# Fannovel16/stylish-tts

Hardware: AMD Instinct MI355X
Metric: utterances_per_sec (higher is better)
Workload: dtype f32; 1 GPU; cfg2: LJSpeech-shaped batch=8 x 3.0 s per GPU (T=240 mel frames, 72000 samples @24 kHz) fp32, Decoder + PriorEncoder/reverse flow + freegan iSTFT vocoder (stts_frame_path); no diffusion step exists in the reference; batch_per_gpu=8, global_batch=8, frames_per_utt=960, parallelism=single GPU, ranks=1, backend=none, distinct_devices=1

## Files before the change

### stylish_tts_amd/csrc/model.hip.h

```cpp
#pragma once
#include <math.h>

#include <array>
#include <map>
#include <memory>
#include <mutex>
#include <string>
#include <vector>

#include "../../include/stylish_hip.h"
#include "common.h"
#include "elementwise.hip.h"
#include "gemm.hip.h"
#include "gemm16.hip.h"
#include "signal.hip.h"
#include "signal_geom.hip.h"
#include "phoneme.hip.h"
#include "wn_layer.hip.h"
#include "wn_layer_small.hip.h"
#include "wn_fused.hip.h"
#include "wn_fused16.hip.h"
#include "wn_block16.hip.h"
#include "wn_fused_x3.hip.h"
#include "wn_block_x3.hip.h"
// ... 742 lines not shown
}
#define STTS_DRY_RETURN(arena)                                                   \
  do {                                                                            \
    if (stts::dry_run().on) {                                                     \
      stts::dry_run().peak = std::max(stts::dry_run().peak, (arena).offset0 + (arena).used); \
      return 0;                                                                   \
    }                                                                             \
  } while (0)

struct Arena {
  char* base;
  size_t cap, used = 0;
  size_t offset0 = 0;
  bool ok = true;
  Arena(void* p, size_t n, size_t off0 = 0) : base((char*)p), cap(n), offset0(off0) {}
  template <typename T>
  T* get(size_t count) {
    const size_t bytes = (count * sizeof(T) + 255) / 256 * 256;
    if (used + bytes > cap) {
      ok = false;
      return nullptr;
    }
    T* p = (T*)(base + used);
    used += bytes;
    return p;
  }
};

struct Seg {
  int n_utt;
  const int* host;
  const int* dev;
  bool cap = false;
  const int* rows_dev() const { return cap ? dev + n_utt : nullptr; }
  int rows() const { return host[n_utt]; }
  int max_len() const {
    int m = 0;
    for (int i = 0; i < n_utt; ++i) m = std::max(m, host[i + 1] - host[i]);
    return m;
  }
};

inline GemmArgs gemm_args(const Seg& s) {
  GemmArgs a;
  memset(&a, 0, sizeof(a));
  a.seg_off = s.dev;
  a.seg_host = s.host;
  a.n_utt = s.n_utt;
  a.rows_total = s.rows();
  a.capacity = s.cap;
  if (!s.cap && s.host && s.n_utt > 0) {
    const int len = s.host[1] - s.host[0];
    bool same = len > 0;
    for (int u = 1; u < s.n_utt && same; ++u) same = s.host[u + 1] - s.host[u] == len;
    if (same) { a.uniform_len = len; a.uniform_lo0 = s.host[0]; }
  }
  a.alpha = 1.0f;
  a.xaff_slope = 0.2f;
  a.zeros = zero_page();
  return a;
}
inline void set_seg(GemmArgs& a, int i, const float* X, int ldx, int xcol0, const PackedConv& w, int pad = -1, int dil = 1) {
  GemmSeg& g = a.seg[i];
  g.X = X;
  g.W = w.W;
  g.W16 = w.W16;
  g.w16_plane = w.w16_plane;
  if (i == 0) a.prec = w.prec;
  g.w_utt_stride = 0;
  g.ldx = ldx;
  g.xcol0 = xcol0;
  g.kc = w.kc;
  g.ntaps = w.ntaps;
  g.dil = dil;
  g.pad = pad >= 0 ? pad : (w.ntaps - 1) / 2;
  g.kreal = w.cin_real;
  if (i == 0) a.wrows = w.rows_real;
  if (a.nseg < i + 1) a.nseg = i + 1;
}

struct WinoScratch {
  float* p = nullptr;
  bool setup = false;
  explicit operator bool() const { return p != nullptr; }
};
inline size_t wino_scratch_floats(const Seg& s, const WinoConv& wc) {
  const long pr = wino_plane_rows(s.rows(), s.n_utt);
  return (size_t)wc.mats.n * pr * (wc.planes.kc * 3 / 2 + round_up(wc.planes.N, 32)) + round_up(s.n_utt + 1 + 16, 32) + 32;
}
template <int N>
inline int run_winograd_n(hipStream_t st, const Seg& s, const float* X, int ldx, const WinoConv& wc, float* Y, int ldy, int act, const float* R, int ldr,
                          float alpha, WinoScratch& scratch, const float* aff = nullptr, int ld_aff = 0, float* stat = nullptr, int ld_stat = 0) {
  const int n = wc.mats.n, kc = wc.planes.kc, ldm = round_up(wc.planes.N, 32), ml = s.max_len();
  long pr = 0;
  for (int u = 0; u < s.n_utt; ++u) pr += ceil_div(s.host[u + 1] - s.host[u], kWinoM);
  const long pr_cap = wino_plane_rows(s.rows(), s.n_utt);
  int* segp = reinterpret_cast<int*>(scratch.p);
  int* goff = segp + 16;
  float* Xp = scratch.p + round_up(s.n_utt + 1 + 16, 32);
  static const bool presplit_env = getenv("STTS_X3_PRESPLIT") && atoi(getenv("STTS_X3_PRESPLIT")) != 0;
  const bool presplit = presplit_env && x3_enabled() && wc.planes.w16_plane > 0 && wc.planes.prec == PREC_F32 && kc % 8 == 0;
  const long xplane = (long)n * pr_cap * kc;
  float* Mp = Xp + (size_t)n * pr_cap * kc * 3 / 2;
  WinoIn ti;
  WinoOut to;
  memcpy(ti.Bt, wc.mats.Bt, sizeof(ti.Bt));
  memcpy(to.At, wc.mats.At, sizeof(to.At));
  const int groups = ceil_div(ml, kWinoM);
  GemmProfiler& prof = gemm_profiler();
  const bool timed = prof.on;
  if (timed) {
    (void)hipEventRecord(prof.next(), st);
    prof.on = false;
  }
  if (!scratch.setup) {
    hipLaunchKernelGGL(wino_setup_kernel, dim3(1), dim3(64), 0, st, s.dev, s.n_utt, kWinoMaxN, goff, segp);
    scratch.setup = true;
  }
  if (presplit)
    hipLaunchKernelGGL((winograd_input_kernel<N, true>), dim3(ceil_div(groups, 4), ceil_div(kc / 4, 64), s.n_utt), dim3(64, 4), 0, st, X, ldx,
                       wc.planes.cin_real, s.dev, wc.pad, ti, Xp, kc, goff, aff, ld_aff, xplane);
  else
  hipLaunchKernelGGL((winograd_input_kernel<N>), dim3(ceil_div(groups, 4), ceil_div(kc / 4, 64), s.n_utt), dim3(64, 4), 0, st, X, ldx,
                     wc.planes.cin_real, s.dev, wc.pad, ti, Xp, kc, goff, aff, ld_aff, 0L);
  std::vector<int> seg_h(n + 1);
  for (int j = 0; j <= n; ++j) seg_h[j] = (int)(j * pr);
  Seg sp{n, seg_h.data(), segp};
  sp.cap = s.cap;
  GemmArgs a = gemm_args(sp);
  set_seg(a, 0, Xp, kc, 0, wc.planes, 0);
  a.seg[0].w_utt_stride = (long)wc.planes.npad * kc;
  if (presplit) {
    a.x16 = 1;
    a.seg[0].x_plane = xplane;
  }
  a.N = wc.planes.N; a.bias = nullptr; a.Y = Mp; a.ldy = ldm;
  {
    const int rc = launch_conv_gemm(st, a, EPI_STORE, wc.planes.npad, n, (int)pr);
    if (rc) {
      prof.on = timed;
      return rc;
    }
  }
  if (stat)
    hipLaunchKernelGGL((winograd_output_kernel<N, true>), dim3(ceil_div(groups, 4), ceil_div(ceil_div(wc.planes.N, 4), 64), s.n_utt), dim3(64, 4), 0, st, Mp, ldm, goff,
                       s.dev, to, wc.planes.bias, act, R, ldr, alpha, Y, ldy, wc.planes.N, stat, ld_stat, ceil_div(groups, 4));
  else
    hipLaunchKernelGGL((winograd_output_kernel<N, false>), dim3(ceil_div(groups, 4), ceil_div(ceil_div(wc.planes.N, 4), 64), s.n_utt), dim3(64, 4), 0, st, Mp, ldm, goff,
                       s.dev, to, wc.planes.bias, act, R, ldr, alpha, Y, ldy, wc.planes.N, nullptr, 0, 0);
  if (timed) {
    prof.on = true;
    (void)hipEventRecord(prof.next(), st);
    prof.add((x3_enabled() && wc.planes.w16_plane > 0) ? "winograd_conv_x3" : "winograd_conv", 0, 2.0 * (double)s.rows() * wc.planes.rows_real * wc.planes.cin_real * wc.mats.r,
             2.0 * (double)n * (double)pr * wc.planes.rows_real * wc.planes.cin_real, 0.0);
  }
  STTS_HIP(hipGetLastError());
  return 0;
}
inline int wino_stat_chunks(const Seg& s) { return ceil_div(ceil_div(s.max_len(), kWinoM), 4); }
inline int run_winograd(hipStream_t st, const Seg& s, const float* X, int ldx, const WinoConv& wc, float* Y, int ldy, int act, const float* R, int ldr,
                        float alpha, WinoScratch& scratch, const float* aff = nullptr, int ld_aff = 0, float* stat = nullptr, int ld_stat = 0) {
  STTS_CHECK(wc.ready && (wc.mats.n == 8 || wc.mats.n == 12), "winograd conv not packed");
  STTS_CHECK(ldx % 4 == 0 && ldy % 4 == 0 && (!R || ldr % 4 == 0), "winograd conv: leading dimensions must be multiples of 4");
  STTS_CHECK(!stat || (ld_stat % 4 == 0 && ld_stat >= round_up(wc.planes.N, 4)), "winograd conv: statistics rows of %d floats do not cover %d channels", ld_stat, wc.planes.N);
  return wc.mats.n == 8 ? run_winograd_n<8>(st, s, X, ldx, wc, Y, ldy, act, R, ldr, alpha, scratch, aff, ld_aff, stat, ld_stat)
                        : run_winograd_n<12>(st, s, X, ldx, wc, Y, ldy, act, R, ldr, alpha, scratch, aff, ld_aff, stat, ld_stat);
}

inline int run_style(hipStream_t st, const StyleTable& t, const float* style, int n_utt, float* out) {
  if (n_utt >= 16 && t.K % 4 == 0 && t.K <= 128) {
    STTS_LAUNCH_PROF("style_fc_batch_kernel", (size_t)t.J * (t.K + n_utt) * 4, style_fc_batch_kernel, dim3(ceil_div(t.J, 4)), dim3(256), st, t.W, t.b, style, out,
                     t.J, t.K, n_utt, t.K, t.ld());
    STTS_HIP(hipGetLastError());
    return 0;
  }
  STTS_LAUNCH_PROF("style_fc_kernel", (size_t)t.J * (t.K + n_utt) * 4, style_fc_kernel, dim3(ceil_div(t.J, 4)), dim3(256), st, t.W, t.b, style, out, t.J, t.K, n_utt, t.K, t.ld());
  STTS_HIP(hipGetLastError());
  return 0;
}

inline dim3 rows_grid(const Seg& s, int per_row_work) {
  const long total = (long)s.max_len() * per_row_work;
  return dim3((unsigned)std::min<long>(std::max<long>(1, ceil_div((int)std::min<long>(total, 1 << 30), 256)), 512), s.n_utt);
}

inline long rows16_threshold() {
  static const long v = getenv("STTS_ROWS16") ? atol(getenv("STTS_ROWS16")) : 3840;
  return v;
}

inline size_t adain_part_floats(const Seg& s, int C, int chunk_rows = kStatChunk) { return (size_t)s.n_utt * ceil_div(s.max_len(), chunk_rows) * 2 * round_up(C, 32); }
inline int run_adain(hipStream_t st, const Seg& s, const float* X, int ldx, int C, float* Y, int ldy, const float* style_out, int ld_style,
                     int gcol0, int act, const float* alpha, float* part, int out16 = 0, bool have_stats = false) {
  const int nchunk = ceil_div(s.max_len(), kStatChunk), ldp = round_up(C, 32);
  if (!have_stats)
    STTS_LAUNCH_PROF("adain_partial_kernel", (size_t)s.rows() * C * 4, adain_partial_kernel, dim3(ceil_div(C, 32), nchunk, s.n_utt), dim3(256), st, X, ldx, C, s.dev, part, ldp, nchunk, kStatChunk);
  const int rb = (long)ceil_div(ldy, 64) * ceil_div(s.rows(), 64) >= 4096 ? 256 : 64;
  STTS_LAUNCH_PROF("adain_apply_kernel", (size_t)s.rows() * (C * 4 + ldy * (out16 ? 2 : 4)), adain_apply_kernel, dim3(ceil_div(ldy, 64), ceil_div(s.max_len(), rb), s.n_utt), dim3(256), st, X, ldx, Y, ldy, C, s.dev,
                     part, ldp, nchunk, style_out, ld_style, gcol0, 1e-5f, act, alpha, out16, rb);
  STTS_HIP(hipGetLastError());
  return 0;
}

struct PendingReduce {
  SplitSrc src{};
  float* Y = nullptr;
  int ldy = 0;
};
inline void pending_from(PendingReduce* p, const SplitInfo& info, const GemmArgs& a) {
  p->src = SplitSrc{};
  if (info.ksplit > 1) {
    p->src = SplitSrc{info.partial, info.ksplit, info.slice_rows, info.ld_part, a.N, a.bias, a.act, a.R, a.ldr, a.rcol0, a.alpha};
    p->Y = a.Y + a.ycol0;
    p->ldy = a.ldy;
  }
}
inline int pending_finish(hipStream_t st, PendingReduce* p) {
  if (!p || !p->src.partial) return 0;
  const SplitSrc& r = p->src;
  const long work = (long)r.slice_rows * ((r.N + 3) / 4);
  STTS_LAUNCH_PROF("splitk_reduce_kernel", (size_t)work * 4 * 4 * (r.ksplit + 1), splitk_reduce_kernel, dim3((unsigned)std::min<long>(2048, (work + 255) / 256)), dim3(256), st, r.partial,
                   r.ksplit, r.slice_rows, 0, r.ld_part, r.N, r.bias, r.act, r.R, r.ldr, r.rcol0, r.alpha, p->Y, p->ldy, 0);
  p->src = SplitSrc{};
  STTS_HIP(hipGetLastError());
  return 0;
}
inline long fold_rows() {
  static const long v = getenv("STTS_FOLD_ROWS") ? atol(getenv("STTS_FOLD_ROWS")) : 2500;
  return v;
}
struct SideWork {
  hipStream_t stream = nullptr;
  hipEvent_t fork = nullptr, join = nullptr;
  float* out = nullptr;
};
struct AdainStats {
  float* in = nullptr;
  bool in_ready = false;
  float* mid = nullptr;
  float* out = nullptr;
  int out_ld = 0;
  bool out_ready = false;
  int chunk_rows = kStatChunk;
};
inline int run_adain_block(hipStream_t st, const Seg& s, const AdainBlockW& B, const float* style_out, int ld_style, const float* x, int ldx,
                           float* y, int ldy, float* act1, float* hbuf, float* act2, float* ss, int force_tile = 0, WinoScratch* wino = nullptr,
                           unsigned short* xs16 = nullptr, bool xs16_ready = false, unsigned short* y16 = nullptr, int ldy16 = 0,
                           AdainStats* stats = nullptr, PendingReduce* pend_in = nullptr, PendingReduce* pend_out = nullptr, const SideWork* side = nullptr) {
  const int ml = s.max_len();
  const bool fold = s.rows() <= (B.conv1.prec == PREC_F32 ? fold_rows() : 4096);
  STTS_CHECK(ldx >= B.kcin, "adain block: input leading dimension %d < padded channels %d", ldx, B.kcin);
  static const bool affine_lanes = getenv("STTS_AFFINE_SERIAL") == nullptr;
  auto affine = [&](const float* X, int ld, int C, int ld_aff, int gcol0, float* aff, PendingReduce* pend = nullptr) {
    const int nchunk = ceil_div(ml, kStatChunk), ldp = round_up(C, 32);
    if (pend && pend->src.partial) {
      STTS_LAUNCH_PROF("adain_partial_reduce_kernel", (size_t)s.rows() * C * 4 * (1 + pend->src.ksplit), adain_partial_reduce_kernel, dim3(ceil_div(C, 32), nchunk, s.n_utt), dim3(256), st,
                       const_cast<float*>(X), ld, C, s.dev, ss, ldp, nchunk, pend->src);
      pend->src = SplitSrc{};
    } else
    STTS_LAUNCH_PROF("adain_partial_kernel", (size_t)s.rows() * C * 4, adain_partial_kernel, dim3(ceil_div(C, 32), nchunk, s.n_utt), dim3(256), st, X, ld, C, s.dev, ss, ldp, nchunk, kStatChunk);
    if (affine_lanes)
      STTS_LAUNCH_PROF("adain_affine_lanes_kernel", (size_t)s.n_utt * nchunk * 2 * ldp * 4, adain_affine_lanes_kernel, dim3(ceil_div(ld_aff, 16), s.n_utt), dim3(256), st, ss, ldp, nchunk, s.dev, style_out, ld_style,
                       gcol0, C, 1e-5f, aff, ld_aff, kStatChunk);
    else
    STTS_LAUNCH_PROF("adain_affine_kernel", (size_t)s.n_utt * nchunk * 2 * ldp * 4, adain_affine_kernel, dim3(ceil_div(ld_aff, 64), s.n_utt), dim3(64), st, ss, ldp, nchunk, s.dev, style_out, ld_style, gcol0, C,
                       1e-5f, aff, ld_aff, kStatChunk);
  };
  GemmArgs a = gemm_args(s);
  PendingReduce pend_mid;
  if (pend_in && pend_in->src.partial) STTS_CHECK(pend_in->Y == x && pend_in->ldy == ldx, "adain block: the pending reduce does not belong to this input");
  if (!fold) STTS_TRY(pending_finish(st, pend_in));
  if (fold) {
    affine(x, ldx, B.cin, B.kcin, B.n1.col0, act1, pend_in);
    set_seg(a, 0, x, ldx, 0, B.conv1);
    a.xaff = act1;
    a.ld_xaff = B.kcin;
  }
  const bool wino1 = !fold && wino && *wino && B.w1.ready && force_tile == 0;
  static const bool wino2_sc = getenv("STTS_NO_WINO_CONV2SC") == nullptr;
  const bool wino2 = !fold && wino && *wino && B.w2.ready && (!B.sc.W || wino2_sc) && force_tile == 0;
  const bool wstats = stats && stats->chunk_rows == kWinoStatChunk && wino1 && wino2;
  auto affine_from = [&](const float* part, int C, int ld_aff, int gcol0, float* aff) {
    const int wch = wino_stat_chunks(s), ldp = round_up(C, 32);
    STTS_LAUNCH_PROF("adain_affine_lanes_kernel", (size_t)s.n_utt * wch * 2 * ldp * 4, adain_affine_lanes_kernel, dim3(ceil_div(ld_aff, 16), s.n_utt), dim3(256), st, part, ldp, wch, s.dev, style_out, ld_style,
                     gcol0, C, 1e-5f, aff, ld_aff, kWinoStatChunk);
  };
  const int h16 = (s.rows() >= rows16_threshold() && B.conv1.prec != PREC_F32 && force_tile == 0 && (!B.sc.W || xs16) && ldx % 8 == 0) ? B.conv1.prec : 0;
  const int nchunk = ceil_div(ml, kStatChunk);
  const bool fuse_stats = stats && h16 && !fold && !wino1 && !wino2;
  if (!fold && !wino1) {
    const bool ready = fuse_stats && stats->in_ready;
    STTS_TRY(run_adain(st, s, x, ldx, B.cin, act1, B.kcin, style_out, ld_style, B.n1.col0, ACT_LRELU, nullptr, ready ? stats->in : ss, h16, ready));
    set_seg(a, 0, act1, B.kcin, 0, B.conv1);
    a.x16 = h16 != 0;
  }
  if (stats) stats->out_ready = false;
  a.N = B.cout;
  a.bias = B.conv1.bias;
  a.Y = hbuf;
  a.ldy = B.cout;
  auto shortcut = [&](hipStream_t sst, float* out) -> int {
    GemmArgs g = gemm_args(s);
    set_seg(g, 0, x, ldx, 0, B.sc);
    g.N = B.cout; g.bias = nullptr; g.Y = out; g.ldy = B.cout;
    return launch_conv_gemm(sst, g, EPI_STORE, B.sc.npad, s.n_utt, ml, 0);
  };
  const bool sc_side = side && side->stream && side->out && wino1 && wino2 && B.sc.W && !gemm_profiler().on;
  if (sc_side) {
    STTS_HIP(hipEventRecord(side->fork, st));
    STTS_HIP(hipStreamWaitEvent(side->stream, side->fork, 0));
    const int rc = shortcut(side->stream, side->out);
    STTS_HIP(hipEventRecord(side->join, side->stream));
    if (rc) { (void)hipStreamWaitEvent(st, side->join, 0); return rc; }
  }
  if (wino1) {
    if (wstats && stats->in_ready) affine_from(stats->in, B.cin, B.kcin, B.n1.col0, act1);
    else affine(x, ldx, B.cin, B.kcin, B.n1.col0, act1);
    STTS_TRY(run_winograd(st, s, x, ldx, B.w1, hbuf, B.cout, ACT_NONE, nullptr, 0, 1.0f, *wino, act1, B.kcin, wstats ? stats->mid : nullptr, round_up(B.cout, 32)));
  } else {
    if (fuse_stats && gemm16_will_run(a, EPI_STORE, B.conv1.npad, s.n_utt)) {
      a.stat_part = stats->mid; a.ld_stat = round_up(B.cout, 32); a.stat_nchunk = nchunk;
    }
    SplitInfo info1{};
    if (fold) a.defer = &info1;
    STTS_TRY(launch_conv_gemm(st, a, EPI_STORE, B.conv1.npad, s.n_utt, ml, force_tile));
    if (fold) pending_from(&pend_mid, info1, a);
  }
  const bool mid_ready = a.stat_part != nullptr;
  GemmArgs b = gemm_args(s);
  if (fold) {
    affine(hbuf, B.cout, B.cout, B.cout, B.n2.col0, act2, &pend_mid);
    set_seg(b, 0, hbuf, B.cout, 0, B.conv2);
    b.xaff = act2;
    b.ld_xaff = B.cout;
  } else if (wino2) {
    if (wstats) affine_from(stats->mid, B.cout, B.cout, B.n2.col0, act2);
    else affine(hbuf, B.cout, B.cout, B.cout, B.n2.col0, act2);
  } else {
    STTS_TRY(run_adain(st, s, hbuf, B.cout, B.cout, act2, B.cout, style_out, ld_style, B.n2.col0, ACT_LRELU, nullptr, mid_ready ? stats->mid : ss, h16, mid_ready));
    set_seg(b, 0, act2, B.cout, 0, B.conv2);
    b.x16 = h16 != 0;
  }
  if (B.sc.W) {
    if (h16) {
      if (!xs16_ready) launch_cast_rows(st, h16, x, ldx, B.cin, xs16, ldx, s.rows());
      set_seg(b, 1, reinterpret_cast<const float*>(xs16), ldx, 0, B.sc);
    } else {
      set_seg(b, 1, x, ldx, 0, B.sc);
    }
  } else {
    b.R = x;
    b.ldr = ldx;
  }
  b.N = B.cout;
  b.bias = B.conv2.bias;
  b.Y = y;
  b.ldy = ldy;
  b.alpha = 0.70710678118654752440f;
  const bool y16_epi = y16 && h16 && !wino2;
  if (y16_epi) {
    b.Y16 = y16;
    b.ldy16 = ldy16;
  }
  if (wino2) {
    const float* res = x;
    int ld_res = ldx;
    if (B.sc.W && sc_side) {
      STTS_HIP(hipStreamWaitEvent(st, side->join, 0));
      res = side->out;
      ld_res = B.cout;
    } else if (B.sc.W) {
      STTS_TRY(shortcut(st, act1));
      res = act1;
      ld_res = B.cout;
    }
    const bool leave = wstats && stats->out;
    STTS_TRY(run_winograd(st, s, hbuf, B.cout, B.w2, y, ldy, ACT_NONE, res, ld_res, b.alpha, *wino, act2, B.cout, leave ? stats->out : nullptr, leave ? stats->out_ld : 0));
    if (leave) stats->out_ready = true;
  } else {
    if (fuse_stats && stats->out && gemm16_will_run(b, EPI_STORE, B.conv2.npad, s.n_utt)) {
      b.stat_part = stats->out; b.ld_stat = stats->out_ld; b.stat_nchunk = nchunk;
      stats->out_ready = true;
    }
    SplitInfo info2{};
    if (fold && pend_out && !y16) b.defer = &info2;
    STTS_TRY(launch_conv_gemm(st, b, EPI_STORE, B.conv2.npad, s.n_utt, ml, force_tile));
    if (fold && pend_out && !y16) pending_from(pend_out, info2, b);
  }
  if (y16 && !y16_epi) launch_cast_rows(st, B.conv1.prec, y, ldy, B.cout, y16, ldy16, s.rows(), B.cout);
  STTS_HIP(hipGetLastError());
  return 0;
}

inline int decoder_forward(stts_ctx* c, hipStream_t st, const Seg& s, const float* asr, int ld_asr, const float* pitch, const float* energy,
                           const float* style, float* x_out, int ld_x, Arena& ws, const SideWork* side_lane = nullptr) {
  const stts_model_dims& d = c->d;
  const long R = s.rows();
  const int ccat = d.dec_hidden + d.dec_residual + 2, ldcat = c->dec[1].kcin;
  const int cenc = d.inter_dim + 2, ldenc = c->dec[0].kcin;
  STTS_CHECK(ldcat >= ccat && ldenc >= cenc, "decoder_forward: packed widths %d / %d do not cover %d / %d channels", ldcat, ldenc, ccat, cenc);
  const int ldwide = std::max(ldenc, ldcat);
  float* enc_in = ws.get<float>(R * ldenc);
  float* xa = ws.get<float>(R * ldcat);
  float* xb = ws.get<float>(R * ldcat);
  float* act1 = ws.get<float>(R * ldwide);
  float* hbuf = ws.get<float>(R * d.dec_hidden);
  float* act2 = ws.get<float>(R * d.dec_hidden);
  float* ss = ws.get<float>(adain_part_floats(s, ldwide));
  float* ss_in = ws.get<float>(adain_part_floats(s, ldwide, kWinoStatChunk));
  float* ss_mid = ws.get<float>(adain_part_floats(s, ldwide, kWinoStatChunk));
  float* sty = ws.get<float>((size_t)s.n_utt * c->dec_style.ld());
  WinoScratch wino;
  if (R > fold_rows() && c->dec[1].w1.ready) wino.p = ws.get<float>(wino_scratch_floats(s, c->dec[1].w1));
  float* sc_out = wino.p && c->dec[1].sc.W ? ws.get<float>(R * d.dec_hidden) : nullptr;
  const bool x16 = R >= rows16_threshold() && c->prec != PREC_F32 && d.dec_hidden % 8 == 0;
  unsigned short* xs16a = x16 ? ws.get<unsigned short>(R * ldwide) : nullptr;
  unsigned short* xs16b = x16 ? ws.get<unsigned short>(R * ldwide) : nullptr;
  STTS_CHECK(ws.ok, "decoder_forward: workspace too small");
  STTS_DRY_RETURN(ws);
  STTS_TRY(run_style(st, c->dec_style, style, s.n_utt, sty));
  FrontArgs fa;
  fa.asr = asr; fa.ld_asr = ld_asr; fa.pitch = pitch; fa.energy = energy;
  for (int i = 0; i < 3; ++i) { fa.wf[i] = c->front_wf[i]; fa.wn[i] = c->front_wn[i]; }
  fa.bf = c->front_bf; fa.bn = c->front_bn;
  fa.enc_in = enc_in; fa.ld_enc = ldenc; fa.xa = xa; fa.xb = xb; fa.ld_x = ldcat;
  fa.c_asr = d.inter_dim; fa.c_hidden = d.dec_hidden; fa.c_res = d.dec_residual;
  STTS_LAUNCH_PROF("decoder_front_kernel", (size_t)R * (d.inter_dim + 2 + ldenc + 2 * 4) * 4, decoder_front_kernel, rows_grid(s, ldenc / 4), dim3(256), st, fa, s.dev);
  for (float* dst : {xa, xb}) {
    GemmArgs a = gemm_args(s);
    set_seg(a, 0, asr, ld_asr, 0, c->asr_res);
    a.N = d.dec_residual; a.bias = c->asr_res.bias; a.Y = dst; a.ldy = ldcat; a.ycol0 = d.dec_hidden;
    STTS_TRY(launch_conv_gemm(st, a, EPI_STORE, c->asr_res.npad, s.n_utt, s.max_len()));
  }
  const int lds = c->dec_style.ld();
  const int ctail = d.dec_hidden & ~7, ntail = ldcat - ctail;
  auto cast_tail = [&](const float* src, unsigned short* dst) {
    launch_cast_rows(st, c->prec, src + ctail, ldcat, ccat - ctail, dst + ctail, ldcat, R, ntail);
  };
  static const bool no_stat_fuse = getenv("STTS_NO_STAT_FUSE") != nullptr;
  static const bool no_wino_stats = getenv("STTS_NO_WINO_STATS") != nullptr;
  const bool wstat_mode = c->prec == PREC_F32 && wino && !no_wino_stats;
  const bool use_stats = (x16 && !no_stat_fuse) || wstat_mode;
  AdainStats stats;
  if (wstat_mode) stats.chunk_rows = kWinoStatChunk;
  stats.mid = ss_mid;
  stats.out = ss_in;
  stats.out_ld = round_up(ccat, 32);
  PendingReduce pend;
  STTS_TRY(run_adain_block(st, s, c->dec[0], sty, lds, enc_in, ldenc, xa, ldcat, act1, hbuf, act2, ss, 0, &wino, xs16b, false, xs16a, ldcat, use_stats ? &stats : nullptr,
                           nullptr, &pend));
  if (x16) {
    cast_tail(xa, xs16a);
    cast_tail(xb, xs16b);
  }
  bool const_ready = false;
  auto const_columns = [&]() -> int {
    if (!stats.out_ready || const_ready) return 0;
    const int nchunk = ceil_div(s.max_len(), stats.chunk_rows), cc0 = d.dec_hidden, ncst = ccat - cc0;
    STTS_CHECK(cc0 % 32 == 0, "decoder_forward: hidden_dim must be a multiple of 32");
    STTS_LAUNCH_PROF("adain_partial_kernel", (size_t)R * ncst * 4, adain_partial_kernel, dim3(ceil_div(ncst, 32), nchunk, s.n_utt), dim3(256), st, xa + cc0, ldcat, ncst, s.dev,
                     ss_in + cc0, stats.out_ld, nchunk, stats.chunk_rows);
    const_ready = true;
    return 0;
  };
  STTS_TRY(const_columns());
  float* cur = xa;
  float* nxt = xb;
  unsigned short* cur16 = xs16a;
  unsigned short* nxt16 = xs16b;
  static const long sc_side_min_rows = getenv("STTS_SC_SIDE_MIN_ROWS") ? atol(getenv("STTS_SC_SIDE_MIN_ROWS")) : 12000;
  SideWork side;
  if (side_lane && sc_out && R >= sc_side_min_rows) {
    side = *side_lane;
    side.out = sc_out;
  }
  auto blocks = [&]() -> int {
    for (int i = 1; i <= 4; ++i) {
      float* dst = i == 4 ? x_out : nxt;
      const int ldd = i == 4 ? ld_x : ldcat;
      STTS_TRY(const_columns());
      stats.in = ss_in;
      stats.in_ready = stats.out_ready;
      stats.out = i == 4 ? nullptr : ss_in;
      STTS_TRY(run_adain_block(st, s, c->dec[i], sty, lds, cur, ldcat, dst, ldd, act1, hbuf, act2, ss, 0, &wino, cur16, x16, i == 4 ? nullptr : nxt16, ldcat,
                               use_stats ? &stats : nullptr, &pend, &pend, side.stream ? &side : nullptr));
      std::swap(cur, nxt);
      std::swap(cur16, nxt16);
    }
    return 0;
  };
  const int rc = blocks();
  if (rc && side.stream) {
    (void)hipEventRecord(side.join, side.stream);
    (void)hipStreamWaitEvent(st, side.join, 0);
  }
  if (rc) return rc;
  return pending_finish(st, &pend);
}

}

#include "flow.hip.h"

namespace stts {


inline int harmonic_stft(stts_ctx* c, hipStream_t st, const Seg& s, const float* pitch, const float* noise, const float* init_phase,
                         int batch_scope, float* prior_out, float* har_spec, float* har_phase, int ld, Arena& ws, int out16 = 0) {
  const long R = s.rows();
  double* prefix = ws.get<double>(R);
  float* stats = ws.get<float>(2 * s.n_utt);
  const SignalGeom& g = c->geom;
  float* sig = prior_out ? prior_out : ws.get<float>(R * g.h);
  STTS_CHECK(ws.ok, "harmonic_stft: workspace too small");
  if (g.generic) STTS_CHECK(ld >= g.bins, "harmonic_stft: row stride %d < %d bins", ld, g.bins);
  else STTS_CHECK(ld >= kBins && ld <= 64 * ((kBins + 63) / 64), "harmonic_stft: row stride %d outside [%d, %d]", ld, kBins, 64 * ((kBins + 63) / 64));
  STTS_DRY_RETURN(ws);
  if (!s.cap)
    for (int u = 0; u < s.n_utt; ++u)
      STTS_CHECK((long)(s.host[u + 1] - s.host[u]) * g.h > g.n_fft / 2, "utterance %d too short for reflect padding (%d frames; need > %d samples)", u,
                 s.host[u + 1] - s.host[u], g.n_fft / 2);
  if (g.generic) {
    STTS_TRY(launch_pcph_geom(st, g, s.n_utt, s.dev, R, s.max_len(), pitch, noise, init_phase, batch_scope, prefix, stats, sig, c->d_err));
    STTS_TRY(launch_stft_geom(st, g, s.n_utt, s.dev, R, s.max_len(), sig, c->hann, c->twiddle64, har_spec, har_phase, ld, out16));
    STTS_HIP(hipGetLastError());
    return 0;
  }
  STTS_LAUNCH_PROF("pcph_prep_kernel", (size_t)R * 12, pcph_prep_kernel, dim3(s.n_utt), dim3(256), st, pitch, s.dev, prefix, stats);
  STTS_LAUNCH_PROF("pcph_kernel", (size_t)R * kHop * 8, pcph_kernel, dim3(std::min(1024, ceil_div(s.max_len() * kHop, 256)), s.n_utt), dim3(256), st, pitch, s.dev, s.n_utt,
                     prefix, stats, noise, init_phase, batch_scope, sig, c->d_err);
  STTS_LAUNCH_PROF("stft_kernel", (size_t)R * (kHop + 2 * kBins) * 4, stft_kernel, dim3((s.max_len() + kFftWaves - 1) / kFftWaves, s.n_utt), dim3(64 * kFftWaves), st, sig, s.dev, c->hann, c->twiddle64, har_spec, har_phase, ld, out16);
  STTS_HIP(hipGetLastError());
  return 0;
}

inline int ln_launch(hipStream_t st, const float* X, int ldx, int C, long n_rows, const int* row_utt, float eps, int adaptive, int nout,
                     const LnOut& o0, const LnOut& o1, int act, const LnIn& in = LnIn{}, const int* n_rows_dev = nullptr) {
  STTS_LAUNCH_PROF("row_layernorm_kernel", (size_t)n_rows * C * (1 + nout) * 4, row_layernorm_kernel, dim3((unsigned)ceil_div((int)n_rows, 4)), dim3(256), st, X, ldx, C, (int)n_rows, row_utt, eps,
                     adaptive, nout, o0, o1, act, in, n_rows_dev);
  STTS_HIP(hipGetLastError());
  return 0;
}

struct ConvNextScratch {
  float *dw, *nrm, *U, *part;
  int ss_stride;
  float *gscale, *w2u;
  const int* row_utt;
};

inline int convnext_block_forward(hipStream_t st, const Seg& s, const ConvNextW& B, int h, int inter, const float* sty, int lds, int p16, const float* cur,
                                  float* nxt, const ConvNextScratch& sc) {
  const long R = s.rows();
  const int ml = s.max_len();
  float *dw = sc.dw, *nrm = sc.nrm, *U = sc.U, *part = sc.part, *gscale = sc.gscale, *w2u = sc.w2u;
  const int ss_stride = sc.ss_stride;
  const int* row_utt = sc.row_utt;
  if (h <= kDwLnMaxC && h % 4 == 0 && (B.K == 3 || B.K == 7 || B.K == 15 || B.K == 31)) {
    const dim3 fg(ceil_div(ml, 16), s.n_utt);
    const size_t fb = (size_t)R * h * (4 + (p16 ? 2 : 4));
#define STTS_DWLN(KK) STTS_LAUNCH_PROF("dwconv_ln_kernel", fb, (dwconv_ln_kernel<KK, 16>), fg, dim3(256), st, cur, h, h, s.dev, B.dw_wt, B.dw_b, 1e-6f, sty, lds, B.norm.col0, nrm, h, p16)
    if (B.K == 3) STTS_DWLN(3);
    else if (B.K == 7) STTS_DWLN(7);
    else if (B.K == 15) STTS_DWLN(15);
    else STTS_DWLN(31);
#undef STTS_DWLN
// ... 301 lines not shown
```

### stylish_tts_amd/csrc/winograd.hip.h

```cpp
#pragma once
#include <array>
#include <cmath>
#include <vector>

#include "gemm.hip.h"

namespace stts {

constexpr int kWinoM = 6;
constexpr int kWinoMaxN = 12;

struct WinoMats {
  int r = 0, n = 0;
  float Bt[kWinoMaxN][kWinoMaxN];
  float At[kWinoM][kWinoMaxN];
  double G[kWinoMaxN][8];
};

inline std::vector<double> wino_polymul(const std::vector<double>& a, const std::vector<double>& b) {
  std::vector<double> c(a.size() + b.size() - 1, 0.0);
  for (size_t i = 0; i < a.size(); ++i)
    for (size_t j = 0; j < b.size(); ++j) c[i + j] += a[i] * b[j];
  return c;
}
// ... 141 lines not shown
  const bool live = g < groups && n4 < Nout;
  if (!STATS && !live) return;
  if (STATS && (int)blockIdx.x * kWinoStatChunk >= len) return;
  f32x4 o[kWinoM];
#pragma unroll
  for (int i = 0; i < kWinoM; ++i) o[i] = f32x4{0.f, 0.f, 0.f, 0.f};
  if (live) {
    const long prow = goff[u] + g, plane_rows = goff[gridDim.z];
    f32x4 m[N];
#pragma unroll
    for (int j = 0; j < N; ++j) m[j] = *reinterpret_cast<const f32x4*>(Mp + ((long)j * plane_rows + prow) * ldm + n4);
    f32x4 b = {0.f, 0.f, 0.f, 0.f};
    if (bias) b = *reinterpret_cast<const f32x4*>(bias + n4);
#pragma unroll
    for (int i = 0; i < kWinoM; ++i) {
      const int row = g * kWinoM + i;
      if (row < len) {
        f32x4 v = b;
#pragma unroll
        for (int j = 0; j < N; ++j) v += t.At[i][j] * m[j];
        float* y = Y + (long)(lo + row) * ldy + n4;
        if (n4 + 4 <= Nout) {
          f32x4 e;
#pragma unroll
          for (int c = 0; c < 4; ++c) e[c] = act_apply(v[c], act);
          if (R) e += *reinterpret_cast<const f32x4*>(R + (long)(lo + row) * ldr + n4);
          e *= alpha;
          *reinterpret_cast<f32x4*>(y) = e;
          o[i] = e;
        } else {
#pragma unroll
          for (int c = 0; c < 4; ++c) {
            if (n4 + c < Nout) {
              float e = act_apply(v[c], act);
              if (R) e += R[(long)(lo + row) * ldr + n4 + c];
              e *= alpha;
              y[c] = e;
              o[i][c] = e;
            }
          }
        }
      }
    }
  }
  if (STATS) {
    __shared__ f32x4 red[2][4][64];
    const int gn = min(kWinoM, max(0, len - g * kWinoM));
    f32x4 gmean = {0.f, 0.f, 0.f, 0.f}, gm2 = {0.f, 0.f, 0.f, 0.f};
    if (gn > 0) {
#pragma unroll
      for (int i = 0; i < kWinoM; ++i) gmean += o[i];
      gmean *= 1.0f / (float)gn;
#pragma unroll
      for (int i = 0; i < kWinoM; ++i) {
        if (i < gn) {
          const f32x4 dv = o[i] - gmean;
          gm2 += dv * dv;
        }
      }
    }
    red[0][threadIdx.y][threadIdx.x] = gmean;
    red[1][threadIdx.y][threadIdx.x] = gm2;
    __syncthreads();
    if (threadIdx.y == 0 && n4 < Nout) {
      const int base = (int)blockIdx.x * kWinoStatChunk;
      const int nrows = min(kWinoStatChunk, len - base);
      f32x4 mean = {0.f, 0.f, 0.f, 0.f};
#pragma unroll
      for (int w = 0; w < 4; ++w) mean += (float)min(kWinoM, max(0, len - base - w * kWinoM)) * red[0][w][threadIdx.x];
      mean *= 1.0f / (float)nrows;
      f32x4 m2 = {0.f, 0.f, 0.f, 0.f};
#pragma unroll
      for (int w = 0; w < 4; ++w) {
        const f32x4 dv = red[0][w][threadIdx.x] - mean;
        m2 += red[1][w][threadIdx.x] + (float)min(kWinoM, max(0, len - base - w * kWinoM)) * dv * dv;
      }
      float* p = stat + ((long)(u * stat_nchunk + blockIdx.x) * 2) * ld_stat + n4;
      *reinterpret_cast<f32x4*>(p) = mean;
      *reinterpret_cast<f32x4*>(p + ld_stat) = m2;
    }
  }
}

}
```

Measured before the change: 2407 utt/s.

## Fuse Winograd output, AdaIN statistics/affine, and next conv input transform into bridge kernel

Adds a winograd_bridge_kernel that takes one Winograd conv's GEMM output planes, does the output transform, bias and residual, computes per-utterance instance-norm statistics, applies the AdaIN affine and LeakyReLU, and writes the next conv's Winograd input planes, all inside one block per 16-channel slab. In the decoder's AdaIN blocks, the separate output, affine, and input-transform kernels are skipped when this bridge path is enabled. The aim is to cut kernel launches and the round trips of intermediate activations through global memory. In exchange each block does more serial work in large thread blocks, and the path only runs for F(6,3) convs, utterances short enough, and a block count inside a fixed range.

```diff
diff --git a/stylish_tts_amd/csrc/model.hip.h b/stylish_tts_amd/csrc/model.hip.h
--- a/stylish_tts_amd/csrc/model.hip.h
+++ b/stylish_tts_amd/csrc/model.hip.h
@@ -848,7 +848,12 @@
 struct WinoScratch {
   float* p = nullptr;
   bool setup = false;
+  int mp_kc = 0;
   explicit operator bool() const { return p != nullptr; }
+};
+struct WinoForm {
+  bool planes_ready = false;
+  bool stop = false;
 };
 inline size_t wino_scratch_floats(const Seg& s, const WinoConv& wc) {
   const long pr = wino_plane_rows(s.rows(), s.n_utt);
@@ -856,7 +861,7 @@
 }
 template <int N>
 inline int run_winograd_n(hipStream_t st, const Seg& s, const float* X, int ldx, const WinoConv& wc, float* Y, int ldy, int act, const float* R, int ldr,
-                          float alpha, WinoScratch& scratch, const float* aff = nullptr, int ld_aff = 0, float* stat = nullptr, int ld_stat = 0) {
+                          float alpha, WinoScratch& scratch, const float* aff = nullptr, int ld_aff = 0, float* stat = nullptr, int ld_stat = 0, WinoForm form = WinoForm{}) {
   const int n = wc.mats.n, kc = wc.planes.kc, ldm = round_up(wc.planes.N, 32), ml = s.max_len();
   long pr = 0;
   for (int u = 0; u < s.n_utt; ++u) pr += ceil_div(s.host[u + 1] - s.host[u], kWinoM);
@@ -866,8 +871,9 @@
   float* Xp = scratch.p + round_up(s.n_utt + 1 + 16, 32);
   static const bool presplit_env = getenv("STTS_X3_PRESPLIT") && atoi(getenv("STTS_X3_PRESPLIT")) != 0;
   const bool presplit = presplit_env && x3_enabled() && wc.planes.w16_plane > 0 && wc.planes.prec == PREC_F32 && kc % 8 == 0;
+  STTS_CHECK(!(form.planes_ready || form.stop || scratch.mp_kc) || (!presplit && scratch.mp_kc >= kc), "winograd conv: chained form with pre-split planes or without a common plane layout");
   const long xplane = (long)n * pr_cap * kc;
-  float* Mp = Xp + (size_t)n * pr_cap * kc * 3 / 2;
+  float* Mp = Xp + (size_t)n * pr_cap * (scratch.mp_kc ? scratch.mp_kc : kc) * 3 / 2;
   WinoIn ti;
   WinoOut to;
   memcpy(ti.Bt, wc.mats.Bt, sizeof(ti.Bt));
@@ -883,7 +889,8 @@
     hipLaunchKernelGGL(wino_setup_kernel, dim3(1), dim3(64), 0, st, s.dev, s.n_utt, kWinoMaxN, goff, segp);
     scratch.setup = true;
   }
-  if (presplit)
+  if (form.planes_ready) {
+  } else if (presplit)
     hipLaunchKernelGGL((winograd_input_kernel<N, true>), dim3(ceil_div(groups, 4), ceil_div(kc / 4, 64), s.n_utt), dim3(64, 4), 0, st, X, ldx,
                        wc.planes.cin_real, s.dev, wc.pad, ti, Xp, kc, goff, aff, ld_aff, xplane);
   else
@@ -908,7 +915,8 @@
       return rc;
     }
   }
-  if (stat)
+  if (form.stop) {
+  } else if (stat)
     hipLaunchKernelGGL((winograd_output_kernel<N, true>), dim3(ceil_div(groups, 4), ceil_div(ceil_div(wc.planes.N, 4), 64), s.n_utt), dim3(64, 4), 0, st, Mp, ldm, goff,
                        s.dev, to, wc.planes.bias, act, R, ldr, alpha, Y, ldy, wc.planes.N, stat, ld_stat, ceil_div(groups, 4));
   else
@@ -925,12 +933,50 @@
 }
 inline int wino_stat_chunks(const Seg& s) { return ceil_div(ceil_div(s.max_len(), kWinoM), 4); }
 inline int run_winograd(hipStream_t st, const Seg& s, const float* X, int ldx, const WinoConv& wc, float* Y, int ldy, int act, const float* R, int ldr,
-                        float alpha, WinoScratch& scratch, const float* aff = nullptr, int ld_aff = 0, float* stat = nullptr, int ld_stat = 0) {
+                        float alpha, WinoScratch& scratch, const float* aff = nullptr, int ld_aff = 0, float* stat = nullptr, int ld_stat = 0, WinoForm form = WinoForm{}) {
   STTS_CHECK(wc.ready && (wc.mats.n == 8 || wc.mats.n == 12), "winograd conv not packed");
   STTS_CHECK(ldx % 4 == 0 && ldy % 4 == 0 && (!R || ldr % 4 == 0), "winograd conv: leading dimensions must be multiples of 4");
   STTS_CHECK(!stat || (ld_stat % 4 == 0 && ld_stat >= round_up(wc.planes.N, 4)), "winograd conv: statistics rows of %d floats do not cover %d channels", ld_stat, wc.planes.N);
-  return wc.mats.n == 8 ? run_winograd_n<8>(st, s, X, ldx, wc, Y, ldy, act, R, ldr, alpha, scratch, aff, ld_aff, stat, ld_stat)
-                        : run_winograd_n<12>(st, s, X, ldx, wc, Y, ldy, act, R, ldr, alpha, scratch, aff, ld_aff, stat, ld_stat);
+  return wc.mats.n == 8 ? run_winograd_n<8>(st, s, X, ldx, wc, Y, ldy, act, R, ldr, alpha, scratch, aff, ld_aff, stat, ld_stat, form)
+                        : run_winograd_n<12>(st, s, X, ldx, wc, Y, ldy, act, R, ldr, alpha, scratch, aff, ld_aff, stat, ld_stat, form);
+}
+
+inline bool wino_bridge_fits(const Seg& s, const WinoConv& A, const WinoConv& Bc, int W) {
+  return A.ready && Bc.ready && A.mats.n == 8 && Bc.mats.n == 8 && Bc.pad == 1 && A.planes.N % W == 0 && Bc.planes.kc % W == 0 && Bc.planes.kc >= A.planes.N &&
+         W == 16 && ceil_div(s.max_len(), kWinoM) <= kWinoBridgeGroups;
+}
+inline int run_wino_bridge(hipStream_t st, const Seg& s, const WinoConv& A, const float* R, int ldr, float alpha, float* Y, int ldy, const WinoConv& Bc,
+                           const float* gb, int ld_gb, int gcol0, int C, const float* part, int ldpart, const float* Xc, int ldxc, WinoScratch& scratch, int W) {
+  STTS_CHECK(wino_bridge_fits(s, A, Bc, W), "winograd bridge: unsupported convs or utterance length");
+  STTS_CHECK(scratch.setup && scratch.mp_kc >= Bc.planes.kc && scratch.mp_kc >= A.planes.kc, "winograd bridge: the scratch holds no planes in the common layout");
+  STTS_CHECK(Bc.planes.kc == A.planes.N || (part && Xc && ldxc % 4 == 0), "winograd bridge: constant columns without statistics or rows");
+  STTS_CHECK((!R || ldr % 4 == 0) && (!Y || ldy % 4 == 0) && C <= Bc.planes.kc && C >= A.planes.N, "winograd bridge: bad leading dimensions or channel count");
+  const long pr_cap = wino_plane_rows(s.rows(), s.n_utt);
+  WinoBridge a;
+  memset(&a, 0, sizeof(a));
+  int* segp = reinterpret_cast<int*>(scratch.p);
+  float* Xp = scratch.p + round_up(s.n_utt + 1 + 16, 32);
+  a.Mp = Xp + (size_t)A.mats.n * pr_cap * scratch.mp_kc * 3 / 2;
+  a.ldm = round_up(A.planes.N, 32);
+  a.bias = A.planes.bias; a.act = ACT_NONE; a.R = R; a.ldr = ldr; a.alpha = alpha; a.Y = Y; a.ldy = ldy; a.Nout = A.planes.N;
+  a.gb = gb; a.ld_gb = ld_gb; a.gcol0 = gcol0; a.C = C; a.eps = 1e-5f;
+  a.part = part; a.ldpart = ldpart; a.nchunk = wino_stat_chunks(s); a.Xc = Xc; a.ldxc = ldxc;
+  a.Xp = Xp; a.kc = Bc.planes.kc;
+  a.goff = segp + 16; a.seg_off = s.dev;
+  memcpy(a.to.At, A.mats.At, sizeof(a.to.At));
+  memcpy(a.ti.Bt, Bc.mats.Bt, sizeof(a.ti.Bt));
+  const dim3 grid(Bc.planes.kc / W, s.n_utt), block(std::max(256, round_up(ceil_div(s.max_len(), kWinoM) * (W / 4), 64)));
+  GemmProfiler& prof = gemm_profiler();
+  hipEvent_t e0 = nullptr, e1 = nullptr;
+  if (prof.on) {
+    e0 = prof.next();
+    e1 = prof.next();
+    prof.add((x3_enabled() && Bc.planes.w16_plane > 0) ? "winograd_conv_x3" : "winograd_conv", 0, 0.0, 0.0, 0.0);
+  }
+  if (e0) hipExtLaunchKernelGGL((winograd_bridge_kernel<8, 16>), grid, block, 0, st, e0, e1, 0, a);
+  else hipLaunchKernelGGL((winograd_bridge_kernel<8, 16>), grid, block, 0, st, a);
+  STTS_HIP(hipGetLastError());
+  return 0;
 }
 
 inline int run_style(hipStream_t st, const StyleTable& t, const float* style, int n_utt, float* out) {
@@ -995,6 +1041,23 @@
   static const long v = getenv("STTS_FOLD_ROWS") ? atol(getenv("STTS_FOLD_ROWS")) : 2500;
   return v;
 }
+constexpr int kBridgeSlab = 16;
+constexpr int kBridgeMinBlocks = 96, kBridgeMaxBlocks = 384;
+inline int adain_bridge_slab(const Seg& s, const AdainBlockW* blocks, int nblocks) {
+  const char* env = getenv("STTS_ADAIN_BRIDGE");
+  const int forced = env ? (atoi(env) != 0) : -1;
+  if (forced == 0) return 0;
+  if (getenv("STTS_X3_PRESPLIT") && atoi(getenv("STTS_X3_PRESPLIT")) != 0) return 0;
+  const int slab = kBridgeSlab;
+  for (int i = 0; i < nblocks; ++i) {
+    const AdainBlockW& B = blocks[i];
+    if (!wino_bridge_fits(s, B.w1, B.w2, slab) || B.w2.planes.kc != B.cout) return 0;
+    if (i + 1 < nblocks && (!wino_bridge_fits(s, B.w2, blocks[i + 1].w1, slab) || blocks[i + 1].cin < B.cout)) return 0;
+  }
+  if (forced == 1) return slab;
+  const long nb = (long)s.n_utt * (blocks[0].cout / slab);
+  return nb >= kBridgeMinBlocks && nb <= kBridgeMaxBlocks ? slab : 0;
+}
 struct SideWork {
   hipStream_t stream = nullptr;
   hipEvent_t fork = nullptr, join = nullptr;
@@ -1008,6 +1071,11 @@
   int out_ld = 0;
   bool out_ready = false;
   int chunk_rows = kStatChunk;
+  int bridge_w = 0;
+  const AdainBlockW* next = nullptr;
+  const float* cst = nullptr;
+  int cst_ld = 0;
+  bool planes_ready = false;
 };
 inline int run_adain_block(hipStream_t st, const Seg& s, const AdainBlockW& B, const float* style_out, int ld_style, const float* x, int ldx,
                            float* y, int ldy, float* act1, float* hbuf, float* act2, float* ss, int force_tile = 0, WinoScratch* wino = nullptr,
@@ -1046,6 +1114,7 @@
   static const bool wino2_sc = getenv("STTS_NO_WINO_CONV2SC") == nullptr;
   const bool wino2 = !fold && wino && *wino && B.w2.ready && (!B.sc.W || wino2_sc) && force_tile == 0;
   const bool wstats = stats && stats->chunk_rows == kWinoStatChunk && wino1 && wino2;
+  const int bw = wstats ? stats->bridge_w : 0;
   auto affine_from = [&](const float* part, int C, int ld_aff, int gcol0, float* aff) {
     const int wch = wino_stat_chunks(s), ldp = round_up(C, 32);
     STTS_LAUNCH_PROF("adain_affine_lanes_kernel", (size_t)s.n_utt * wch * 2 * ldp * 4, adain_affine_lanes_kernel, dim3(ceil_div(ld_aff, 16), s.n_utt), dim3(256), st, part, ldp, wch, s.dev, style_out, ld_style,
@@ -1080,9 +1149,14 @@
     if (rc) { (void)hipStreamWaitEvent(st, side->join, 0); return rc; }
   }
   if (wino1) {
+    if (bw && stats->planes_ready) {
+      STTS_TRY(run_winograd(st, s, nullptr, 0, B.w1, nullptr, 0, ACT_NONE, nullptr, 0, 1.0f, *wino, nullptr, 0, nullptr, 0, WinoForm{true, true}));
+    } else {
     if (wstats && stats->in_ready) affine_from(stats->in, B.cin, B.kcin, B.n1.col0, act1);
     else affine(x, ldx, B.cin, B.kcin, B.n1.col0, act1);
-    STTS_TRY(run_winograd(st, s, x, ldx, B.w1, hbuf, B.cout, ACT_NONE, nullptr, 0, 1.0f, *wino, act1, B.kcin, wstats ? stats->mid : nullptr, round_up(B.cout, 32)));
+    STTS_TRY(run_winograd(st, s, x, ldx, B.w1, hbuf, B.cout, ACT_NONE, nullptr, 0, 1.0f, *wino, act1, B.kcin, wstats && !bw ? stats->mid : nullptr, round_up(B.cout, 32),
+                          WinoForm{false, bw != 0}));
+    }
   } else {
     if (fuse_stats && gemm16_will_run(a, EPI_STORE, B.conv1.npad, s.n_utt)) {
       a.stat_part = stats->mid; a.ld_stat = round_up(B.cout, 32); a.stat_nchunk = nchunk;
@@ -1100,7 +1174,8 @@
     b.xaff = act2;
     b.ld_xaff = B.cout;
   } else if (wino2) {
-    if (wstats) affine_from(stats->mid, B.cout, B.cout, B.n2.col0, act2);
+    if (bw) {
+    } else if (wstats) affine_from(stats->mid, B.cout, B.cout, B.n2.col0, act2);
     else affine(hbuf, B.cout, B.cout, B.cout, B.n2.col0, act2);
   } else {
     STTS_TRY(run_adain(st, s, hbuf, B.cout, B.cout, act2, B.cout, style_out, ld_style, B.n2.col0, ACT_LRELU, nullptr, mid_ready ? stats->mid : ss, h16, mid_ready));
@@ -1139,6 +1214,15 @@
       STTS_TRY(shortcut(st, act1));
       res = act1;
       ld_res = B.cout;
+    }
+    if (bw) {
+      STTS_TRY(run_wino_bridge(st, s, B.w1, nullptr, 0, 1.0f, nullptr, 0, B.w2, style_out, ld_style, B.n2.col0, B.cout, nullptr, 0, nullptr, 0, *wino, bw));
+      const AdainBlockW* nb = stats->next;
+      STTS_TRY(run_winograd(st, s, nullptr, 0, B.w2, y, ldy, ACT_NONE, res, ld_res, b.alpha, *wino, nullptr, 0, nullptr, 0, WinoForm{true, nb != nullptr}));
+      if (nb) STTS_TRY(run_wino_bridge(st, s, B.w2, res, ld_res, b.alpha, y, ldy, nb->w1, style_out, ld_style, nb->n1.col0, nb->cin, stats->cst, stats->cst_ld, y, ldy, *wino, bw));
+      stats->planes_ready = nb != nullptr;
+      STTS_HIP(hipGetLastError());
+      return 0;
     }
     const bool leave = wstats && stats->out;
     STTS_TRY(run_winograd(st, s, hbuf, B.cout, B.w2, y, ldy, ACT_NONE, res, ld_res, b.alpha, *wino, act2, B.cout, leave ? stats->out : nullptr, leave ? stats->out_ld : 0));
@@ -1212,16 +1296,17 @@
   stats.mid = ss_mid;
   stats.out = ss_in;
   stats.out_ld = round_up(ccat, 32);
+  const int bridge_w = wstat_mode ? adain_bridge_slab(s, c->dec, 5) : 0;
+  if (bridge_w) {
+    stats.bridge_w = bridge_w;
+    stats.cst = ss_in;
+    stats.cst_ld = stats.out_ld;
+    wino.mp_kc = c->dec[1].w1.planes.kc;
+  }
   PendingReduce pend;
-  STTS_TRY(run_adain_block(st, s, c->dec[0], sty, lds, enc_in, ldenc, xa, ldcat, act1, hbuf, act2, ss, 0, &wino, xs16b, false, xs16a, ldcat, use_stats ? &stats : nullptr,
-                           nullptr, &pend));
-  if (x16) {
-    cast_tail(xa, xs16a);
-    cast_tail(xb, xs16b);
-  }
   bool const_ready = false;
   auto const_columns = [&]() -> int {
-    if (!stats.out_ready || const_ready) return 0;
+    if (!(stats.out_ready || bridge_w) || const_ready) return 0;
     const int nchunk = ceil_div(s.max_len(), stats.chunk_rows), cc0 = d.dec_hidden, ncst = ccat - cc0;
     STTS_CHECK(cc0 % 32 == 0, "decoder_forward: hidden_dim must be a multiple of 32");
     STTS_LAUNCH_PROF("adain_partial_kernel", (size_t)R * ncst * 4, adain_partial_kernel, dim3(ceil_div(ncst, 32), nchunk, s.n_utt), dim3(256), st, xa + cc0, ldcat, ncst, s.dev,
@@ -1229,6 +1314,17 @@
     const_ready = true;
     return 0;
   };
+  if (bridge_w) {
+    STTS_CHECK(c->dec[0].cout == d.dec_hidden, "decoder_forward: the blocks' width %d is not hidden_dim %d", c->dec[0].cout, d.dec_hidden);
+    STTS_TRY(const_columns());
+    stats.next = &c->dec[1];
+  }
+  STTS_TRY(run_adain_block(st, s, c->dec[0], sty, lds, enc_in, ldenc, xa, ldcat, act1, hbuf, act2, ss, 0, &wino, xs16b, false, xs16a, ldcat, use_stats ? &stats : nullptr,
+                           nullptr, &pend));
+  if (x16) {
+    cast_tail(xa, xs16a);
+    cast_tail(xb, xs16b);
+  }
   STTS_TRY(const_columns());
   float* cur = xa;
   float* nxt = xb;
@@ -1248,6 +1344,7 @@
       stats.in = ss_in;
       stats.in_ready = stats.out_ready;
       stats.out = i == 4 ? nullptr : ss_in;
+      stats.next = bridge_w && i < 4 ? &c->dec[i + 1] : nullptr;
       STTS_TRY(run_adain_block(st, s, c->dec[i], sty, lds, cur, ldcat, dst, ldd, act1, hbuf, act2, ss, 0, &wino, cur16, x16, i == 4 ? nullptr : nxt16, ldcat,
                                use_stats ? &stats : nullptr, &pend, &pend, side.stream ? &side : nullptr));
       std::swap(cur, nxt);
diff --git a/stylish_tts_amd/csrc/winograd.hip.h b/stylish_tts_amd/csrc/winograd.hip.h
--- a/stylish_tts_amd/csrc/winograd.hip.h
+++ b/stylish_tts_amd/csrc/winograd.hip.h
@@ -247,4 +247,213 @@
   }
 }
 
-}
+constexpr int kWinoBridgeGroups = 256;
+struct WinoBridge {
+  const float* Mp;
+  int ldm;
+  const float* bias;
+  int act;
+  const float* R;
+  int ldr;
+  float alpha;
+  float* Y;
+  int ldy, Nout;
+  const float* gb;
+  int ld_gb, gcol0, C;
+  float eps;
+  const float* part;
+  int ldpart, nchunk;
+  const float* Xc;
+  int ldxc;
+  float* Xp;
+  int kc;
+  const int* goff;
+  const int* seg_off;
+  WinoOut to;
+  WinoIn ti;
+};
+
+template <int N>
+__device__ __forceinline__ void wino_bridge_rows(const WinoBridge& a, int lo, int len, long plane_rows, long prow, int g, int n4, bool write, f32x4 (&o)[kWinoM]) {
+  f32x4 m[N];
+#pragma unroll
+  for (int j = 0; j < N; ++j) m[j] = *reinterpret_cast<const f32x4*>(a.Mp + ((long)j * plane_rows + prow) * a.ldm + n4);
+  f32x4 b = {0.f, 0.f, 0.f, 0.f};
+  if (a.bias) b = *reinterpret_cast<const f32x4*>(a.bias + n4);
+#pragma unroll
+  for (int i = 0; i < kWinoM; ++i) {
+    const int row = g * kWinoM + i;
+    if (row < len) {
+      f32x4 v = b;
+#pragma unroll
+      for (int j = 0; j < N; ++j) v += a.to.At[i][j] * m[j];
+      f32x4 e;
+#pragma unroll
+      for (int c = 0; c < 4; ++c) e[c] = act_apply(v[c], a.act);
+      if (a.R) e += *reinterpret_cast<const f32x4*>(a.R + (long)(lo + row) * a.ldr + n4);
+      e *= a.alpha;
+      if (write) *reinterpret_cast<f32x4*>(a.Y + (long)(lo + row) * a.ldy + n4) = e;
+      o[i] = e;
+    }
+  }
+}
+__device__ __forceinline__ float wino_bridge_mean_part(const float* p0, int ldp, int nch, int len, int lane) {
+  float acc = 0.f;
+#pragma unroll 4
+  for (int ch = lane; ch < nch; ch += 16) {
+    const float nc = (float)min(kWinoStatChunk, len - ch * kWinoStatChunk);
+    acc += nc * p0[(long)ch * 2 * ldp];
+  }
+  return acc;
+}
+__device__ __forceinline__ float wino_bridge_m2_part(const float* p0, int ldp, int nch, int len, int lane, float mean) {
+  float acc = 0.f;
+#pragma unroll 4
+  for (int ch = lane; ch < nch; ch += 16) {
+    const float nc = (float)min(kWinoStatChunk, len - ch * kWinoStatChunk);
+    const float* p = p0 + (long)ch * 2 * ldp;
+    const float d = p[0] - mean;
+    acc += p[ldp] + nc * d * d;
+  }
+  return acc;
+}
+
+template <int N, int W>
+__global__ void __launch_bounds__(1024) winograd_bridge_kernel(const WinoBridge a) {
+  static_assert(N == 8 && W == 16, "F(6,3), slabs of 16 channels (the merge below is adain_affine_lanes_kernel's block: 16 channels x 16 lanes)");
+  constexpr int L = W / 4;
+  __shared__ f32x4 red[2][1024];
+  __shared__ float tab[(kWinoBridgeGroups / 4) * 2 * W];
+  __shared__ float mred[16][17];
+  __shared__ float s_sc[W], s_sh[W];
+  const int u = blockIdx.y, tid = threadIdx.x;
+  const int lo = a.seg_off[u], len = a.seg_off[u + 1] - lo;
+  const int groups = (len + kWinoM - 1) / kWinoM;
+  if (groups * L > (int)blockDim.x) return;
+  const bool cst = (int)blockIdx.x * W >= a.Nout;
+  const int ln = tid % L, g = tid / L;
+  const int c4 = (int)blockIdx.x * W + ln * 4;
+  const long plane_rows = a.goff[gridDim.y], prow0 = a.goff[u];
+  const bool live = g < groups;
+  f32x4 d[N];
+#pragma unroll
+  for (int q = 0; q < N; ++q) d[q] = f32x4{0.f, 0.f, 0.f, 0.f};
+  if (!cst) {
+    f32x4 o[kWinoM];
+#pragma unroll
+    for (int i = 0; i < kWinoM; ++i) o[i] = f32x4{0.f, 0.f, 0.f, 0.f};
+    if (live) wino_bridge_rows<N>(a, lo, len, plane_rows, prow0 + g, g, c4, a.Y != nullptr, o);
+    const int gn = min(kWinoM, max(0, len - g * kWinoM));
+    f32x4 gmean = {0.f, 0.f, 0.f, 0.f}, gm2 = {0.f, 0.f, 0.f, 0.f};
+    if (gn > 0) {
+#pragma unroll
+      for (int i = 0; i < kWinoM; ++i) gmean += o[i];
+      gmean *= 1.0f / (float)gn;
+#pragma unroll
+      for (int i = 0; i < kWinoM; ++i) {
+        if (i < gn) {
+          const f32x4 dv = o[i] - gmean;
+          gm2 += dv * dv;
+        }
+      }
+    }
+    red[0][tid] = gmean;
+    red[1][tid] = gm2;
+    __syncthreads();
+    const int base = (g >> 2) * kWinoStatChunk;
+    if ((g & 3) == 0 && base < len) {
+      const int nrows = min(kWinoStatChunk, len - base);
+      f32x4 mean = {0.f, 0.f, 0.f, 0.f};
+#pragma unroll
+      for (int w = 0; w < 4; ++w) mean += (float)min(kWinoM, max(0, len - base - w * kWinoM)) * red[0][tid + w * L];
+      mean *= 1.0f / (float)nrows;
+      f32x4 m2 = {0.f, 0.f, 0.f, 0.f};
+#pragma unroll
+      for (int w = 0; w < 4; ++w) {
+        const f32x4 dv = red[0][tid + w * L] - mean;
+        m2 += red[1][tid + w * L] + (float)min(kWinoM, max(0, len - base - w * kWinoM)) * dv * dv;
+      }
+      *reinterpret_cast<f32x4*>(tab + ((g >> 2) * 2) * W + ln * 4) = mean;
+      *reinterpret_cast<f32x4*>(tab + ((g >> 2) * 2 + 1) * W + ln * 4) = m2;
+    }
+    __syncthreads();
+#pragma unroll
+    for (int i = 0; i < kWinoM; ++i) d[i + 1] = o[i];
+  } else if (live) {
+#pragma unroll
+    for (int q = 0; q < N; ++q) {
+      const int row = g * kWinoM - 1 + q;
+      if (row >= 0 && row < len && c4 < a.C) d[q] = *reinterpret_cast<const f32x4*>(a.Xc + (long)(lo + row) * a.ldxc + c4);
+    }
+  }
+  {
+    const int cl = tid & 15, lane = (tid >> 4) & 15;
+    const bool mt = tid < 256;
+    const int nch = (len + kWinoStatChunk - 1) / kWinoStatChunk;
+    const int c = (int)blockIdx.x * W + cl;
+    const bool ok = c < a.C;
+    const float* pg = a.part + ((long)u * a.nchunk * 2) * a.ldpart + (ok ? c : 0);
+    float acc = 0.f;
+    if (mt) acc = cst ? wino_bridge_mean_part(pg, a.ldpart, nch, len, lane) : wino_bridge_mean_part(tab + cl, W, nch, len, lane);
+    if (mt) mred[lane][cl] = acc;
+    __syncthreads();
+    float mean = 0.f;
+#pragma unroll
+    for (int i = 0; i < 16; ++i) mean += mred[i][cl];
+    mean /= (float)len;
+    __syncthreads();
+    if (mt) acc = cst ? wino_bridge_m2_part(pg, a.ldpart, nch, len, lane, mean) : wino_bridge_m2_part(tab + cl, W, nch, len, lane, mean);
+    if (mt) mred[lane][cl] = acc;
+    __syncthreads();
+    if (tid < 16) {
+      float sc = 0.f, sh = 0.f;
+      if (ok && len > 0) {
+        float m2 = 0.f;
+#pragma unroll
+        for (int i = 0; i < 16; ++i) m2 += mred[i][cl];
+        const float rstd = rsqrtf(m2 / (float)len + a.eps);
+        const float gm = a.gb[(long)u * a.ld_gb + a.gcol0 + c], be = a.gb[(long)u * a.ld_gb + a.gcol0 + a.C + c];
+        sc = rstd * (1.0f + gm);
+        sh = be - mean * sc;
+      }
+      s_sc[cl] = sc;
+      s_sh[cl] = sh;
+    }
+    __syncthreads();
+  }
+  const f32x4 sc = *reinterpret_cast<const f32x4*>(s_sc + ln * 4), sh = *reinterpret_cast<const f32x4*>(s_sh + ln * 4);
+#pragma unroll
+  for (int q = 0; q < N; ++q) {
+    const int row = g * kWinoM - 1 + q;
+    const bool in = row >= 0 && row < len && c4 < a.C && (cst || (q > 0 && q < N - 1));
+    if (in) {
+#pragma unroll
+      for (int e = 0; e < 4; ++e) {
+        const float y = (sc[e] == 0.0f ? 0.0f : d[q][e] * sc[e]) + sh[e];
+        d[q][e] = y >= 0.0f ? y : 0.2f * y;
+      }
+    }
+    if (c4 + 3 >= a.C) {
+#pragma unroll
+      for (int e = 1; e < 4; ++e)
+        if (c4 + e >= a.C) d[q][e] = 0.0f;
+    }
+  }
+  if (!cst) {
+    red[0][tid] = d[1];
+    red[1][tid] = d[N - 2];
+    __syncthreads();
+    if (live && g > 0) d[0] = red[1][tid - L];
+    if (live && (g + 1) * kWinoM < len) d[N - 1] = red[0][tid + L];
+  }
+  if (!live) return;
+#pragma unroll
+  for (int j = 0; j < N; ++j) {
+    f32x4 v = {0.f, 0.f, 0.f, 0.f};
+#pragma unroll
+    for (int q = 0; q < N; ++q) v += a.ti.Bt[j][q] * d[q];
+    *reinterpret_cast<f32x4*>(a.Xp + ((long)j * plane_rows + prow0 + g) * a.kc + c4) = v;
+  }
+}
+
+}
```

New measurement: 2436 utt/s, median of 6. 1.01x the previous value.
